# taaha-khan/2023-CompaCT-Image-Compression

Measured on AMD Instinct MI355X. Metric: MPixels/s encode+decode, 12-bit 512x512 CT batch, bytes-exact, higher is better.
Workload: dtype u16

## Files before the change

### 2023-compact-image-compression_amd/csrc/deflate_kernels.hip

```cpp
#include <hip/hip_runtime.h>
#include <cstring>
#include <algorithm>

#include "cct_internal.h"
#include "../../include/compact_hip.h"

namespace cct {
namespace {

constexpr int MIN_MATCH = 3, MAX_MATCH = 258, WSIZE = 32768;
constexpr int MIN_LOOKAHEAD = MAX_MATCH + MIN_MATCH + 1;
constexpr int MAX_DIST = WSIZE - MIN_LOOKAHEAD;
constexpr int TOO_FAR = 4096;
constexpr int BLOCK_SYMS = 16383;
constexpr int BLOCK_SYMS_ML9 = 32767;
constexpr int L_CODES = 286, D_CODES = 30, BL_CODES = 19, HEAP_SIZE = 2 * L_CODES + 1;
constexpr int END_BLOCK = 256, MAX_BITS = 15, MAX_BL_BITS = 7;
constexpr uint32_t Z_FILTERED = 1, Z_HUFFMAN_ONLY = 2, Z_RLE = 3, Z_FIXED = 4;
__host__ __device__ __forceinline__ bool short_pass(uint32_t strategy) { return strategy == Z_HUFFMAN_ONLY || strategy == Z_RLE; }

__constant__ uint8_t c_extra_lbits[29] = {0,0,0,0,0,0,0,0,1,1,1,1,2,2,2,2,3,3,3,3,4,4,4,4,5,5,5,5,0};
__constant__ uint8_t c_extra_dbits[30] = {0,0,0,0,1,1,2,2,3,3,4,4,5,5,6,6,7,7,8,8,9,9,10,10,11,11,12,12,13,13};
__constant__ uint8_t c_extra_blbits[19] = {0,0,0,0,0,0,0,0,0,0,0,0,0,0,0,0,2,3,7};
__constant__ uint8_t c_bl_order[19] = {16,17,18,0,8,7,9,6,10,5,11,4,12,3,13,2,14,1,15};
__constant__ uint8_t c_length_code[256];
__constant__ uint16_t c_base_length[29];
__constant__ uint8_t c_dist_code[512];
__constant__ uint16_t c_base_dist[30];
__constant__ uint16_t c_static_lcode[288];
__constant__ uint8_t c_static_llen[288];
__constant__ uint16_t c_static_dcode[30];

template <int HB>
__device__ __forceinline__ uint32_t hash3(uint32_t b0, uint32_t b1, uint32_t b2)
{
	constexpr int SH = (HB + 2) / 3;
	return ((b0 << (2 * SH)) ^ (b1 << SH) ^ b2) & ((1u << HB) - 1u);
}

__device__ __forceinline__ int d_code(uint32_t dist) { return dist < 256 ? c_dist_code[dist] : c_dist_code[256 + (dist >> 7)]; }

struct MatchRec { uint16_t len_full, len_quarter, dist_full, dist_quarter; };
constexpr uint32_t GEN_MAX = 16383;
__device__ __forceinline__ uint2 pack_match(uint32_t len_full, uint32_t len_quarter, uint32_t dist_full, uint32_t dist_quarter, uint32_t gen)
{
	return make_uint2((len_full | ((gen & 127u) << 9)) | ((len_quarter | ((gen >> 7) << 9)) << 16), dist_full | (dist_quarter << 16));
}
__device__ __forceinline__ MatchRec checked_match(MatchRec r, uint32_t gen, uint32_t rw, uint32_t p, uint32_t L)
{
	const uint32_t tag = (uint32_t)(r.len_full >> 9) | ((uint32_t)(r.len_quarter >> 9) << 7);
	const uint32_t lookahead = L - min(p, L);
	const uint32_t max_len = lookahead < (uint32_t)MAX_MATCH ? lookahead : (uint32_t)MAX_MATCH;
	const bool maximal = (rw >> 15) && (rw & 0x7FFFu) >= max_len && p + 2 < L;
	MatchRec o;
	const bool ok = tag == gen;
	o.len_full = ok ? (uint16_t)(r.len_full & 511u) : (uint16_t)(maximal ? max_len : 0u);
	o.len_quarter = ok ? (uint16_t)(r.len_quarter & 511u) : (uint16_t)(maximal ? max_len : 0u);
	o.dist_full = ok ? r.dist_full : (uint16_t)(maximal ? 1u : 0u);
	o.dist_quarter = ok ? r.dist_quarter : (uint16_t)(maximal ? 1u : 0u);
	return o;
}

__device__ __forceinline__ void lds_barrier()
{
	asm volatile("s_waitcnt lgkmcnt(0)\n\ts_barrier" ::: "memory");
}

__device__ __forceinline__ uint32_t wave_sum(uint32_t v)
{
#pragma unroll
	for (int d = 32; d >= 1; d >>= 1) v += (uint32_t)__shfl_xor((int)v, d, 64);
	return v;
}

template <bool FIRST, int HB>
__global__ void __launch_bounds__(1024) dfl_sort_pass_kernel(DeflateArgs a)
{
	constexpr int BITS = FIRST ? 8 : HB - 8, NB = 1 << BITS;
	constexpr uint32_t HMASK = (1u << HB) - 1u;
	__shared__ uint32_t offs[256];
	__shared__ uint32_t wcnt[16][NB];
	const int s = blockIdx.x;
	const uint32_t L = a.in_sizes[s];
	const uint8_t *in = a.in + (size_t)s * a.in_stride;
	const size_t base = (size_t)s * a.in_stride;
	const uint32_t npos = L >= MIN_MATCH ? L - 2 : 0;
	const uint64_t *rec_src = a.rec_in + base;
	uint64_t *rec_dst = (FIRST ? a.rec_in : a.rec_out) + base;
	const int tid = threadIdx.x, lane = tid & 63, wave = tid >> 6;
	const uint64_t lt_mask = (1ull << lane) - 1ull;
	if (tid < 256) offs[tid] = 0;
	__syncthreads();
	if (tid < NB) offs[tid] = a.sort_hist[(size_t)s * SORT_HIST + (FIRST ? 0 : 256) + tid];
	__syncthreads();
	if (wave == 0) {
		uint32_t v[4], sum = 0;
#pragma unroll
		for (int k = 0; k < 4; k++) { v[k] = offs[lane * 4 + k]; sum += v[k]; }
		uint32_t inc = sum;
#pragma unroll
		for (int d = 1; d < 64; d <<= 1) { const uint32_t o = (uint32_t)__shfl_up((int)inc, d, 64); if (lane >= d) inc += o; }
		uint32_t run = inc - sum;
#pragma unroll
		for (int k = 0; k < 4; k++) { offs[lane * 4 + k] = run; run += v[k]; }
	}
	__syncthreads();
#ifndef CCT_SORT_E
#define CCT_SORT_E 4
#endif
	constexpr int E = CCT_SORT_E;
	constexpr int ND = E / 4;
	const uint32_t last = npos ? npos - 1 : 0;
	static_assert(E % 4 == 0 && ND + 1 <= E, "pass A: whole dwords per lane, kept in ra[0 .. ND]");
#ifdef CCT_SORT_PROBE
	const bool compact = false;
#else
	const bool compact = HB == 15 && a.pos_mask != 0xFFFFFFFFu;
#endif
	const uint32_t dmax = (uint32_t)a.in_stride - 4u;
	auto fetch = [&](uint32_t tile_base, uint32_t (&ra)[E], uint32_t (&rb)[E]) {
		if (FIRST) {
#pragma unroll
			for (int d = 0; d < ND; d++) ra[d] = *reinterpret_cast<const uint32_t *>(in + min(tile_base + 256u * d + 4u * (uint32_t)lane, dmax));
			ra[ND] = *reinterpret_cast<const uint32_t *>(in + min(tile_base + 256u * ND, dmax));
#pragma unroll
			for (int e = 0; e < E; e++) rb[e] = compact ? a.run_len[base + min(tile_base + (uint32_t)(e * 64 + lane), last)] : 0u;
		} else {
#pragma unroll
			for (int e = 0; e < E; e++) {
				const uint64_t r = rec_src[min(tile_base + (uint32_t)(e * 64 + lane), last)];
				ra[e] = (uint32_t)r; rb[e] = (uint32_t)(r >> 32);
			}
		}
	};
	auto finish = [&](uint32_t tile_base, const uint32_t (&ra)[E], const uint32_t (&rb)[E], uint32_t (&h)[E], uint32_t (&p)[E]) {
#pragma unroll
		for (int e = 0; e < E; e++) {
			const uint32_t idx = tile_base + (uint32_t)(e * 64 + lane);
			if (FIRST) {
				const int la = (e & 3) * 16 + (lane >> 2);
				const uint32_t da = (uint32_t)__builtin_amdgcn_ds_bpermute(la << 2, (int)ra[e >> 2]);
				uint32_t db = (uint32_t)__builtin_amdgcn_ds_bpermute(((la + 1) & 63) << 2, (int)ra[e >> 2]);
				if ((e & 3) == 3) {
					const uint32_t nxt = (e >> 2) + 1 < ND ? (uint32_t)__builtin_amdgcn_readfirstlane((int)ra[(e >> 2) + 1 < ND ? (e >> 2) + 1 : 0]) : ra[ND];
					if (la == 63) db = nxt;
				}
				const uint32_t sh = (uint32_t)lane & 3u;
				const uint32_t w = __builtin_amdgcn_alignbyte(db, da, sh);
				const uint32_t b0 = w & 255u, b1 = (w >> 8) & 255u, b2 = (w >> 16) & 255u;
				h[e] = hash3<HB>(b0, b1, b2); p[e] = idx;
				if (compact) {
					const uint32_t b4 = (db >> (8u * sh)) & 255u;
					const uint32_t f16 = (b0 == b1 && b1 == b2) ? rb[e] : ((w >> 24) | (b4 << 8));
					h[e] |= (f16 << 15) | ((b0 >> 7) << 31); p[e] |= (b1 << 22) | (((b0 >> 5) & 3u) << 30);
				}
			}
			else { h[e] = rb[e]; p[e] = ra[e]; }
			if (idx >= npos) { h[e] = 0; p[e] = idx; }
		}
	};
	uint32_t hn[E], pn[E];
	{
		uint32_t ra[E], rb[E];
		fetch((uint32_t)(wave * 64 * E), ra, rb);
		finish((uint32_t)(wave * 64 * E), ra, rb, hn, pn);
	}
	for (uint32_t t0 = 0; t0 < npos; t0 += 1024 * E) {
		uint32_t h[E], p[E], rk[E], ra[E], rb[E];
		const uint32_t idx0 = t0 + (uint32_t)(wave * 64 * E + lane);
#pragma unroll
		for (int e = 0; e < E; e++) { h[e] = hn[e]; p[e] = pn[e]; }
		const uint32_t next_base = t0 + (uint32_t)(1024 * E + wave * 64 * E);
		fetch(next_base, ra, rb);
		for (int k = lane; k < NB; k += 64) wcnt[wave][k] = 0;
#pragma unroll
		for (int e = 0; e < E; e++) {
			const bool valid = idx0 + e * 64 < npos;
			const uint32_t d = FIRST ? (h[e] & 255u) : ((h[e] & HMASK) >> 8);
			uint64_t same = __ballot(valid);
#pragma unroll
			for (int b = 0; b < BITS; b++) {
				const bool bit = (d >> b) & 1u;
				const uint64_t bal = __ballot(bit);
				same &= bit ? bal : ~bal;
			}
			const uint32_t rank = (uint32_t)__popcll(same & lt_mask);
			uint32_t before = 0;
			if (valid) {
				before = wcnt[wave][d];
				if (rank == 0) wcnt[wave][d] = before + (uint32_t)__popcll(same);
			}
			rk[e] = before + rank;
		}
		lds_barrier();
		if (tid < NB) {
			uint32_t c[16], run = offs[tid];
#pragma unroll
			for (int w = 0; w < 16; w++) c[w] = wcnt[w][tid];
#pragma unroll
			for (int w = 0; w < 16; w++) { wcnt[w][tid] = run; run += c[w]; }
			offs[tid] = run;
		}
		lds_barrier();
#pragma unroll
		for (int e = 0; e < E; e++) asm volatile("" : "+v"(ra[e]), "+v"(rb[e]) :: "memory");
		finish(next_base, ra, rb, hn, pn);
#pragma unroll
		for (int e = 0; e < E; e++) {
			if (idx0 + e * 64 < npos) {
				const uint32_t d = FIRST ? (h[e] & 255u) : ((h[e] & HMASK) >> 8);
				const uint32_t dst = wcnt[wave][d] + rk[e];
				rec_dst[dst] = (uint64_t)p[e] | ((uint64_t)h[e] << 32);
			}
		}
	}
}

constexpr int LIGHT_STEPS = 12;

__device__ __forceinline__ bool xcd_slice(int n, int &s, uint32_t &part, uint32_t &nparts)
{
	const uint32_t lin = blockIdx.x + gridDim.x * blockIdx.y;
	const uint32_t c = lin & 7u, k = lin >> 3;
	nparts = gridDim.x;
	s = (int)(8u * (k / nparts) + c);
	part = k % nparts;
	return s < n;
}

__device__ __forceinline__ uint32_t nil_candidate(uint32_t p, uint32_t lookahead)
{
	return (lookahead < (uint32_t)MIN_LOOKAHEAD && p >= 32506u + 32768u && (p - 32506u) % 32768u == 0) ? p - 32506u : 0xFFFFFFFFu;
}

constexpr int RUNLEN_OUT = 2048 - 264;

template <bool SORT, int HB>
__global__ void __launch_bounds__(256) dfl_run_len_kernel(DeflateArgs a)
{
	constexpr int NH = 256 + (1 << (HB - 8));
	__shared__ uint32_t wtot[4];
	__shared__ uint32_t hist[SORT ? NH : 1];
	if (SORT) for (int t = threadIdx.x; t < NH; t += 256) hist[t] = 0;
	__syncthreads();
	const int s = blockIdx.y;
	const uint32_t L = a.in_sizes[s];
	const uint8_t *in = a.in + (size_t)s * a.in_stride;
	uint16_t *rl = a.run_len + (size_t)s * a.in_stride;
	const int lane = threadIdx.x & 63, wave = threadIdx.x >> 6;
	const uint32_t nchunks = (L + RUNLEN_OUT - 1) / RUNLEN_OUT;
	for (uint32_t c = blockIdx.x; c < nchunks; c += gridDim.x) {
		const uint32_t c0 = c * RUNLEN_OUT;
		const uint32_t g = c0 + threadIdx.x * 8;
		uint8_t b[12];
		if (g + 12 <= L && g >= 1) {
			uint64_t w;
			__builtin_memcpy(&w, in + g, 8);
#pragma unroll
			for (int k = 0; k < 8; k++) b[k + 1] = (uint8_t)(w >> (8 * k));
			b[0] = in[g - 1];
			uint32_t w2; __builtin_memcpy(&w2, in + g + 8, 4);
			b[9] = (uint8_t)w2; b[10] = (uint8_t)(w2 >> 8); b[11] = (uint8_t)(w2 >> 16);
		} else {
#pragma unroll
			for (int k = 0; k < 12; k++) { const int64_t y = (int64_t)g - 1 + k; b[k] = (y >= 0 && y < (int64_t)L) ? in[y] : 0; }
		}
		if (SORT) {
			uint32_t hk[8], cnt = 0, h0 = 0;
			bool same = true;
#pragma unroll
			for (int k = 0; k < 8; k++) {
				const bool v = threadIdx.x * 8 + k < (uint32_t)RUNLEN_OUT && g + k + 2 < L;
				hk[k] = v ? hash3<HB>(b[k + 1], b[k + 2], b[k + 3]) : 0xFFFFFFFFu;
				if (v) { if (!cnt) h0 = hk[k]; else same &= hk[k] == h0; cnt++; }
			}
			const bool wave_same = __all(same && cnt == 8 && h0 == (uint32_t)__builtin_amdgcn_readfirstlane((int)h0));
			if (wave_same) {
				if (lane == 0) { atomicAdd(&hist[h0 & 255u], 512u); atomicAdd(&hist[256u + (h0 >> 8)], 512u); }
			} else if (same) {
				if (cnt) { atomicAdd(&hist[h0 & 255u], cnt); atomicAdd(&hist[256u + (h0 >> 8)], cnt); }
			} else {
#pragma unroll
				for (int k = 0; k < 8; k++)
					if (hk[k] != 0xFFFFFFFFu) { atomicAdd(&hist[hk[k] & 255u], 1u); atomicAdd(&hist[256u + (hk[k] >> 8)], 1u); }
			}
		}
		uint32_t chg = 0;
#pragma unroll
		for (int k = 0; k < 8; k++) chg |= (uint32_t)(b[k + 1] != b[k + 2] || g + k + 1 >= L) << k;
		uint32_t hc = chg != 0, n = hc ? (uint32_t)__ffs((int)chg) - 1u : 8u;
#pragma unroll
		for (int d = 1; d < 64; d <<= 1) {
			const uint32_t hb = (uint32_t)__shfl_down((int)hc, d, 64), nb = (uint32_t)__shfl_down((int)n, d, 64);
			if (lane + d < 64 && !hc) { n += nb; hc = hb; }
		}
		__syncthreads();
		if (lane == 0) wtot[wave] = (hc << 31) | n;
		__syncthreads();
		uint32_t xh = 0, xn = 0;
		for (int w = 3; w > wave; w--) {
			const uint32_t t = wtot[w];
			if (t >> 31) { xh = 1; xn = t & 0x7FFFFFFFu; } else xn += t & 0x7FFFFFFFu;
		}
		if (!xh) xn += 1024;
		const uint32_t nfull = hc ? n : n + xn;
		uint32_t nnext = (uint32_t)__shfl_down((int)nfull, 1, 64);
		if (lane == 63) nnext = xn;
		uint16_t out[8];
#pragma unroll
		for (int k = 0; k < 8; k++) {
			const uint32_t rest = chg >> k;
			uint32_t r = rest ? (uint32_t)__ffs((int)rest) : (8u - k) + nnext + 1u;
			if (r > (uint32_t)MAX_MATCH) r = MAX_MATCH;
			out[k] = (uint16_t)(r | ((g + k >= 2 && b[k] == b[k + 1]) ? 0x8000u : 0u));
		}
		if (threadIdx.x * 8 < (uint32_t)RUNLEN_OUT && g < L) {
			if (g + 8 <= L && threadIdx.x * 8 + 8 <= (uint32_t)RUNLEN_OUT) __builtin_memcpy(rl + g, out, 16);
			else {
#pragma unroll
				for (int k = 0; k < 8; k++) if (g + k < L && threadIdx.x * 8 + k < (uint32_t)RUNLEN_OUT) rl[g + k] = out[k];
			}
		}
		if (SORT) {
			uint32_t cx = g == 0 ? 1u : 0u;
#pragma unroll
			for (int i = 0; i < 11; i++) cx |= (uint32_t)(b[i] != b[i + 1] || g + (uint32_t)i >= L) << i;
			const uint32_t t8 = threadIdx.x * 8;
			const uint32_t npub = t8 < (uint32_t)RUNLEN_OUT ? min(min(8u, (uint32_t)RUNLEN_OUT - t8), g < L ? L - g : 0u) : 0u;
			const uint32_t pubm = (1u << npub) - 1u;
			const uint32_t ne3 = g + 3 < L ? min(8u, L - 3u - g) : 0u;
			const uint32_t run3 = ~(cx >> 1) & ~(cx >> 2);
			const uint32_t me = run3 & (cx >> 3) & pubm & ((1u << ne3) - 1u);
			const uint32_t ms = run3 & cx & pubm;
			uint32_t ce = 0, cs = 0;
			if (__any((me | ms) != 0)) { ce = wave_sum((uint32_t)__popc(me)); cs = wave_sum((uint32_t)__popc(ms)); }
			if (lane == 0 && (ce | cs)) {
				uint32_t *cnt = a.run_counts + (size_t)s * 2 * a.run_chunks;
				if (ce) atomicAdd(&cnt[2 * c], ce);
				if (cs) atomicAdd(&cnt[2 * c + 1], cs);
			}
		}
	}
	if (!SORT) return;
	__syncthreads();
	for (int t = threadIdx.x; t < NH; t += 256)
		if (hist[t]) atomicAdd(&a.sort_hist[(size_t)s * SORT_HIST + t], hist[t]);
}

__device__ __forceinline__ int common_prefix(const uint8_t *x, const uint8_t *y, int len, int cap)
{
	while (len + 8 <= cap) {
		uint64_t u, v;
		__builtin_memcpy(&u, x + len, 8);
		__builtin_memcpy(&v, y + len, 8);
		const uint64_t d = u ^ v;
		if (d) return len + ((__ffsll((long long)d) - 1) >> 3);
		len += 8;
	}
	while (len < cap && x[len] == y[len]) len++;
	return len;
}

__device__ __forceinline__ uint32_t rec_hash(uint64_t r, uint32_t pos_mask)
{
	return (uint32_t)(r >> 32) & (pos_mask == 0xFFFFFFFFu ? 0xFFFFFFFFu : 0x7FFFu);
}
__device__ __forceinline__ uint32_t rec_pos(uint64_t r, uint32_t pos_mask) { return (uint32_t)r & pos_mask; }
constexpr uint32_t COMPACT_POS_BITS = 22, COMPACT_POS_MASK = (1u << COMPACT_POS_BITS) - 1u;

__device__ __forceinline__ void light_match_from_memory(const uint8_t *in, const uint64_t *recs, const uint16_t *rl, uint32_t pos_mask,
                                                        uint32_t L, uint32_t i, uint32_t p, uint32_t h, uint32_t nice, int quarter,
                                                        int &kind, int &best, uint32_t &best_q, int &best1, uint32_t &best_q1,
                                                        uint32_t &run_r)
{
	const uint32_t lookahead = L - p;
	const int max_len = lookahead < (uint32_t)MAX_MATCH ? (int)lookahead : MAX_MATCH;
	const int nice_eff = (int)min(lookahead, nice);
	const uint32_t nil_q = nil_candidate(p, lookahead);
	int count = 0;
	const uint8_t *sp = in + p;
	const bool wide = p + 8 <= L;
	uint64_t ow = 0;
	if (wide) __builtin_memcpy(&ow, sp, 8);
	const bool in_run = wide ? (((ow >> 8) ^ ow) & 0xFFFFu) == 0 : (sp[1] == sp[0] && sp[2] == sp[0]);
	if (in_run) {
		const uint32_t rw = rl[p];
		run_r = rw & 0x7FFFu;
		if ((rw >> 15) && (int)run_r >= nice_eff) { best = best1 = (int)run_r; best_q = best_q1 = p - 1; }
		else kind = 2;
		return;
	}
	for (int64_t j = (int64_t)i - 1; j >= 0; j--) {
		const uint64_t rj = recs[j];
		if (rec_hash(rj, pos_mask) != h) break;
		if (count == LIGHT_STEPS) { kind = 1; break; }
		const uint32_t q = rec_pos(rj, pos_mask);
		const uint32_t dist = p - q;
		if (q == 0 || q == nil_q) break;
		if (count == 0 ? dist > (uint32_t)MAX_DIST : dist >= (uint32_t)MAX_DIST) break;
		const uint8_t *mp = in + q;
		{
			int len = 0;
			if (wide) {
				if (best < 8 || mp[best] == sp[best]) {
					uint64_t cw;
					__builtin_memcpy(&cw, mp, 8);
					const uint64_t d = cw ^ ow;
					len = d ? (__ffsll((long long)d) - 1) >> 3 : common_prefix(mp, sp, 8, max_len);
				}
			} else if (mp[best] == sp[best]) len = common_prefix(mp, sp, 0, max_len);
			if (len > best) {
				best = len; best_q = q;
				if (count < quarter) { best1 = len; best_q1 = q; }
			}
		}
		count++;
		if (best >= nice_eff) break;
	}
}

__device__ __forceinline__ uint32_t wave_shift_up(uint32_t v, uint32_t fill)
{
	return (uint32_t)__builtin_amdgcn_update_dpp((int)fill, (int)v, 0x138, 0xF, 0xF, false);
}

template <bool CMP, bool QL>
__global__ void dfl_match_kernel(DeflateArgs a, int n)
{
	int s; uint32_t part, nparts;
	if (!xcd_slice(n, s, part, nparts)) return;
	const uint32_t L = a.in_sizes[s];
	const uint8_t *in = a.in + (size_t)s * a.in_stride;
	const size_t base = (size_t)s * a.in_stride;
	const uint32_t npos = L >= MIN_MATCH ? L - 2 : 0;
	const uint64_t *recs = a.rec_out + base;
	uint2 *mr = reinterpret_cast<uint2 *>(a.mr) + base;
	uint32_t *heavy = a.heavy_list + base;
	const uint16_t *rl = a.run_len + base;
	const int lane = threadIdx.x & 63;
	const uint64_t lt_mask = (1ull << lane) - 1ull;
	const uint32_t gen = *a.gen;
	const int quarter = QL ? (int)(a.max_chain >> 2) : LIGHT_STEPS + 1;
	for (uint32_t i0 = part * blockDim.x; i0 < npos; i0 += nparts * blockDim.x) {
		const uint32_t i = i0 + threadIdx.x;
		const bool valid = i < npos;
		int kind = 0;
		int best = 0, best1 = 0;
		uint32_t best_q = 0, best_q1 = 0, run_r = 0;
		const uint64_t ri = recs[min(i, npos - 1)];
		const uint32_t p = rec_pos(ri, CMP ? COMPACT_POS_MASK : 0xFFFFFFFFu);
		const uint32_t h = rec_hash(ri, CMP ? COMPACT_POS_MASK : 0xFFFFFFFFu);
		bool from_memory = valid;
		bool found = false;
		if (CMP) {
			const uint64_t rb = recs[min(i >= 64 ? i - 64 : 0u, npos - 1)];
			const uint32_t lo_i = (uint32_t)ri, hi_i = (uint32_t)(ri >> 32), lo_b = (uint32_t)rb, hi_b = (uint32_t)(rb >> 32);
			const uint32_t lookahead = L - p;
			const int max_len = lookahead < (uint32_t)MAX_MATCH ? (int)lookahead : MAX_MATCH;
			const int nice_eff = (int)min(lookahead, a.nice);
			const bool fast = valid && p + 8 <= L;
			from_memory = valid && !fast;
			const uint32_t nil_q = nil_candidate(p, lookahead);
			const uint32_t b1 = (lo_i >> 22) & 255u;
			const bool in_run = h == (((b1 << 10) ^ (b1 << 5) ^ b1) & 0x7FFFu) && (((lo_i >> 30) | ((hi_i >> 31) << 2)) == (b1 >> 5));
			if (fast && in_run) {
				const uint32_t rw = (hi_i >> 15) & 0xFFFFu;
				run_r = rw & 0x7FFFu;
				if (!((rw >> 15) && (int)run_r >= nice_eff)) kind = 2;
				else if ((int)run_r < max_len) { best = best1 = (int)run_r; best_q = best_q1 = p - 1; found = true; }
			}
			bool act = fast && !in_run;
			const uint32_t qmin_head = (p > (uint32_t)MAX_DIST ? p - (uint32_t)MAX_DIST : 1u) + (nil_q != 0xFFFFFFFFu ? 1u : 0u);
			const uint32_t qmin_rest = p >= (uint32_t)MAX_DIST ? p - (uint32_t)MAX_DIST + 1u : 1u;
			const uint32_t steps_i = min(i, (uint32_t)LIGHT_STEPS + 1u);
			uint32_t clo = lo_i, chi = hi_i;
#pragma unroll
			for (int k = 1; k <= LIGHT_STEPS + 1; k++) {
				clo = wave_shift_up(clo, (uint32_t)__builtin_amdgcn_readlane((int)lo_b, 64 - k));
				chi = wave_shift_up(chi, (uint32_t)__builtin_amdgcn_readlane((int)hi_b, 64 - k));
				if (!__any(act)) break;
				const uint32_t x = hi_i ^ chi;
				const uint32_t q = clo & COMPACT_POS_MASK;
				if ((uint32_t)k > steps_i || (x & 0x7FFFu) != 0 || q < (k == 1 ? qmin_head : qmin_rest)) act = false;
				if (act) {
					if (k == LIGHT_STEPS + 1) { kind = 1; act = false; }
					else {
						if (best < nice_eff && (((lo_i ^ clo) >> 22) | (x >> 31)) == 0) {
							int len;
							if (x & 0x007F8000u) len = 3;
							else if (x) len = 4;
							else if (best < 5 || in[q + best] == in[p + best]) len = common_prefix(in + q, in + p, 5, max_len);
							else len = 0;
							if (len > best) {
								best = len; best_q = q; found = true;
								if (QL && k <= quarter) { best1 = len; best_q1 = q; }
							}
						}
						if (best >= nice_eff) act = false;
					}
				}
			}
		}
		if (from_memory) {
			light_match_from_memory(in, recs, rl, CMP ? COMPACT_POS_MASK : 0xFFFFFFFFu, L, i, p, h, a.nice, quarter, kind, best, best_q,
			                        best1, best_q1, run_r);
			found = kind == 0 && best >= MIN_MATCH;
		}
		if (found && kind == 0) {
			if (!QL) { best1 = best; best_q1 = best_q; }
			mr[p] = pack_match((uint32_t)best, (uint32_t)best1, p - best_q, best1 ? p - best_q1 : 0u, gen);
		}
		const uint64_t bh = __ballot(kind == 1), br = __ballot(kind == 2);
		uint32_t base_h = 0, base_r = 0;
		if (lane == 0) {
			if (bh) base_h = atomicAdd(&a.heavy_count[s], (uint32_t)__popcll(bh));
			if (br) base_r = atomicAdd(&a.deep_count[s], (uint32_t)__popcll(br));
		}
		base_h = (uint32_t)__shfl((int)base_h, 0, 64); base_r = (uint32_t)__shfl((int)base_r, 0, 64);
// ... 1494 lines not shown
```

Baseline: 16260.

## Specialize radix sort pass on compact flag and streamline wave ranking

The radix sort pass is split into two compile-time versions on the compact-record flag, so the per-element branch inside the inner loops goes away. Per-element validity checks become wave-uniform lane counts, read through readfirstlane. The ballot-based rank now builds its mismatch masks with sbfe sign-extension and XOR and uses an inclusive mask, so that the compiler can keep more values in scalar registers. The scatter now runs before the next tile's finish, with explicit register moves, to reshape the load/compute overlap; the inline asm constraints may add moves or limit scheduling.

```diff
diff --git a/2023-compact-image-compression_amd/csrc/deflate_kernels.hip b/2023-compact-image-compression_amd/csrc/deflate_kernels.hip
--- a/2023-compact-image-compression_amd/csrc/deflate_kernels.hip
+++ b/2023-compact-image-compression_amd/csrc/deflate_kernels.hip
@@ -1,6 +1,7 @@
 #include <hip/hip_runtime.h>
 #include <cstring>
 #include <algorithm>
+#include <type_traits>
 
 #include "cct_internal.h"
 #include "../../include/compact_hip.h"
@@ -81,14 +82,14 @@
 	__shared__ uint32_t offs[256];
 	__shared__ uint32_t wcnt[16][NB];
 	const int s = blockIdx.x;
-	const uint32_t L = a.in_sizes[s];
+	const uint32_t L = (uint32_t)__builtin_amdgcn_readfirstlane((int)a.in_sizes[s]);
 	const uint8_t *in = a.in + (size_t)s * a.in_stride;
 	const size_t base = (size_t)s * a.in_stride;
 	const uint32_t npos = L >= MIN_MATCH ? L - 2 : 0;
 	const uint64_t *rec_src = a.rec_in + base;
-	uint64_t *rec_dst = (FIRST ? a.rec_in : a.rec_out) + base;
-	const int tid = threadIdx.x, lane = tid & 63, wave = tid >> 6;
-	const uint64_t lt_mask = (1ull << lane) - 1ull;
+	uint64_t *rec_dst1 = (FIRST ? a.rec_in : a.rec_out) + base - 1;
+	const int tid = threadIdx.x, lane = tid & 63, wave = __builtin_amdgcn_readfirstlane(tid >> 6);
+	const uint64_t gt_mask = ~1ull << lane, le_mask = ~gt_mask;
 	if (tid < 256) offs[tid] = 0;
 	__syncthreads();
 	if (tid < NB) offs[tid] = a.sort_hist[(size_t)s * SORT_HIST + (FIRST ? 0 : 256) + tid];
@@ -113,12 +114,14 @@
 	const uint32_t last = npos ? npos - 1 : 0;
 	static_assert(E % 4 == 0 && ND + 1 <= E, "pass A: whole dwords per lane, kept in ra[0 .. ND]");
 #ifdef CCT_SORT_PROBE
-	const bool compact = false;
+	const bool compact_records = false;
 #else
-	const bool compact = HB == 15 && a.pos_mask != 0xFFFFFFFFu;
+	const bool compact_records = FIRST && HB == 15 && a.pos_mask != 0xFFFFFFFFu;
 #endif
 	const uint32_t dmax = (uint32_t)a.in_stride - 4u;
-	auto fetch = [&](uint32_t tile_base, uint32_t (&ra)[E], uint32_t (&rb)[E]) {
+	auto valid_lanes = [&](uint32_t first) { return npos - (uint32_t)__builtin_amdgcn_readfirstlane((int)min(npos, first)); };
+	auto fetch = [&](auto compact_c, uint32_t tile_base, uint32_t (&ra)[E], uint32_t (&rb)[E]) {
+		constexpr bool compact = decltype(compact_c)::value;
 		if (FIRST) {
 #pragma unroll
 			for (int d = 0; d < ND; d++) ra[d] = *reinterpret_cast<const uint32_t *>(in + min(tile_base + 256u * d + 4u * (uint32_t)lane, dmax));
@@ -133,7 +136,8 @@
 			}
 		}
 	};
-	auto finish = [&](uint32_t tile_base, const uint32_t (&ra)[E], const uint32_t (&rb)[E], uint32_t (&h)[E], uint32_t (&p)[E]) {
+	auto finish = [&](auto compact_c, uint32_t tile_base, const uint32_t (&ra)[E], const uint32_t (&rb)[E], uint32_t (&h)[E], uint32_t (&p)[E]) {
+		constexpr bool compact = decltype(compact_c)::value;
 #pragma unroll
 		for (int e = 0; e < E; e++) {
 			const uint32_t idx = tile_base + (uint32_t)(e * 64 + lane);
@@ -156,64 +160,75 @@
 				}
 			}
 			else { h[e] = rb[e]; p[e] = ra[e]; }
-			if (idx >= npos) { h[e] = 0; p[e] = idx; }
 		}
 	};
-	uint32_t hn[E], pn[E];
-	{
-		uint32_t ra[E], rb[E];
-		fetch((uint32_t)(wave * 64 * E), ra, rb);
-		finish((uint32_t)(wave * 64 * E), ra, rb, hn, pn);
-	}
-	for (uint32_t t0 = 0; t0 < npos; t0 += 1024 * E) {
-		uint32_t h[E], p[E], rk[E], ra[E], rb[E];
-		const uint32_t idx0 = t0 + (uint32_t)(wave * 64 * E + lane);
-#pragma unroll
-		for (int e = 0; e < E; e++) { h[e] = hn[e]; p[e] = pn[e]; }
-		const uint32_t next_base = t0 + (uint32_t)(1024 * E + wave * 64 * E);
-		fetch(next_base, ra, rb);
-		for (int k = lane; k < NB; k += 64) wcnt[wave][k] = 0;
+	constexpr uint32_t TILE = 1024u * E;
+	const uint32_t wbase = (uint32_t)(wave * 64 * E);
+	auto digit = [&](uint32_t h) { return FIRST ? (h & 255u) : ((h & HMASK) >> 8); };
+	auto rank_tile = [&](uint32_t *row, uint32_t tb, const uint32_t (&h)[E], uint32_t (&rk)[E]) {
+		for (int k = lane; k < NB; k += 64) row[k] = 0;
 #pragma unroll
 		for (int e = 0; e < E; e++) {
-			const bool valid = idx0 + e * 64 < npos;
-			const uint32_t d = FIRST ? (h[e] & 255u) : ((h[e] & HMASK) >> 8);
-			uint64_t same = __ballot(valid);
+			const uint32_t nv = valid_lanes(tb + (uint32_t)(e * 64));
+			const uint64_t inval = nv >= 64u ? 0ull : ~0ull << (nv & 63u);
+			uint32_t dlo = (uint32_t)inval, dhi = (uint32_t)(inval >> 32);
 #pragma unroll
 			for (int b = 0; b < BITS; b++) {
-				const bool bit = (d >> b) & 1u;
-				const uint64_t bal = __ballot(bit);
-				same &= bit ? bal : ~bal;
-			}
-			const uint32_t rank = (uint32_t)__popcll(same & lt_mask);
-			uint32_t before = 0;
-			if (valid) {
-				before = wcnt[wave][d];
-				if (rank == 0) wcnt[wave][d] = before + (uint32_t)__popcll(same);
-			}
-			rk[e] = before + rank;
-		}
-		lds_barrier();
+				const uint32_t m = (uint32_t)__builtin_amdgcn_sbfe(h[e], (FIRST ? 0 : 8) + b, 1);
+				const uint64_t bal = __ballot((int32_t)m < 0);
+				dlo |= (uint32_t)bal ^ m; dhi |= (uint32_t)(bal >> 32) ^ m;
+			}
+			const uint64_t diff = (uint64_t)dlo | ((uint64_t)dhi << 32);
+			uint32_t *cnt = row + digit(h[e]);
+			const uint32_t upto = *cnt + (uint32_t)__popcll(~diff & le_mask);
+			if (diff >= gt_mask) *cnt = upto;
+			rk[e] = upto;
+		}
+	};
+	auto scan_tile = [&](uint32_t (*cnt)[NB]) {
 		if (tid < NB) {
 			uint32_t c[16], run = offs[tid];
 #pragma unroll
-			for (int w = 0; w < 16; w++) c[w] = wcnt[w][tid];
-#pragma unroll
-			for (int w = 0; w < 16; w++) { wcnt[w][tid] = run; run += c[w]; }
+			for (int w = 0; w < 16; w++) c[w] = cnt[w][tid];
+#pragma unroll
+			for (int w = 0; w < 16; w++) { cnt[w][tid] = run; run += c[w]; }
 			offs[tid] = run;
 		}
-		lds_barrier();
-#pragma unroll
-		for (int e = 0; e < E; e++) asm volatile("" : "+v"(ra[e]), "+v"(rb[e]) :: "memory");
-		finish(next_base, ra, rb, hn, pn);
+	};
+	auto scatter_tile = [&](const uint32_t *row, uint32_t tb, const uint32_t (&h)[E], const uint32_t (&p)[E], const uint32_t (&rk)[E]) {
 #pragma unroll
 		for (int e = 0; e < E; e++) {
-			if (idx0 + e * 64 < npos) {
-				const uint32_t d = FIRST ? (h[e] & 255u) : ((h[e] & HMASK) >> 8);
-				const uint32_t dst = wcnt[wave][d] + rk[e];
-				rec_dst[dst] = (uint64_t)p[e] | ((uint64_t)h[e] << 32);
-			}
-		}
-	}
+			if ((uint32_t)lane < valid_lanes(tb + (uint32_t)(e * 64))) {
+				const uint32_t dst = row[digit(h[e])] + rk[e];
+				rec_dst1[dst] = (uint64_t)p[e] | ((uint64_t)h[e] << 32);
+			}
+		}
+	};
+	auto take = [&](uint32_t (&ra)[E], uint32_t (&rb)[E], uint32_t (&qa)[E], uint32_t (&qb)[E]) {
+#pragma unroll
+		for (int e = 0; e < E; e++) {
+			if (!FIRST || e <= ND) asm volatile("v_mov_b32 %0, %1" : "=v"(qa[e]) : "v"(ra[e]) : "memory");
+			else qa[e] = 0;
+			if (!FIRST) asm volatile("v_mov_b32 %0, %1" : "=v"(qb[e]) : "v"(rb[e]) : "memory");
+			else { asm volatile("" : "+v"(rb[e]) :: "memory"); qb[e] = rb[e]; }
+		}
+	};
+	auto sort_tiles = [&](auto compact_c) {
+		uint32_t h[E], p[E], rk[E], ra[E], rb[E], qa[E], qb[E];
+		fetch(compact_c, wbase, ra, rb);
+		finish(compact_c, wbase, ra, rb, h, p);
+		for (uint32_t t0 = 0; t0 < npos; t0 += TILE) {
+			fetch(compact_c, t0 + TILE + wbase, ra, rb);
+			rank_tile(wcnt[wave], t0 + wbase, h, rk);
+			lds_barrier();
+			scan_tile(wcnt);
+			lds_barrier();
+			take(ra, rb, qa, qb);
+			scatter_tile(wcnt[wave], t0 + wbase, h, p, rk);
+			finish(compact_c, t0 + TILE + wbase, qa, qb, h, p);
+		}
+	};
+	if (compact_records) sort_tiles(std::true_type()); else sort_tiles(std::false_type());
 }
 
 constexpr int LIGHT_STEPS = 12;
```

Result: slower. 15960 (-1.8%).
